# intelligent-environments-lab/CityLearn

Hardware: AMD Instinct MI355X
Metric: building-timesteps/sec at 17 bldgs x 65536 envs; HBM GB/s vs roofline (higher is better)
Workload: dtype f32 (battery soc chain in f64); 1 GPU; citylearn_challenge_2022_phase_all tables (17 buildings, the full year, 8 760 h) x 65536 envs per GPU, cl_step_f32 mode A (one env step per launch, state in HBM, fresh uniform random actions from an 8-tensor ring), env batch sharded over GPUs, no collective; CLD_F64_CHAIN: battery soc chain in float64, degraded capacity carried as the capacity loss; envs_per_gpu=65536, buildings=17, env_pitch=65536, precision=CLD_F64_CHAIN (StepEngine default): 1e-4 free-running over whole episodes, launch=hipGraph replay, reward=RewardFunction, reps=1, statistic=median of reps (each: MAX over ranks)

## Files before the change

citylearn_amd/csrc/cl_kernels.hip:

```cpp
#include "cl_trace.h"
#include "cl_unit.h"
#include "cl_plan.h"
#ifndef CL_LEAN_NT_LOADS
#define CL_LEAN_NT_LOADS true
#endif
#include "cl_philox.h"

#include <type_traits>
#include <mutex>
#include <stdarg.h>
#include <string.h>
#include <stdio.h>

namespace {

int hip_fail(hipError_t e, const char* what) {
    return fail(CL_EHIP, "%s: %s", what, hipGetErrorString(e));
}

hipError_t ensure_dynamic_lds(const void* fn, size_t bytes) {
    struct Seen { const void* fn; int dev; size_t bytes; };
    static Seen seen[64];
    static int n_seen = 0;
    static std::mutex mu;
// ... 154 lines not shown
    for (int j = w; j < opw; j += 16) {
        const int o = by * opw + j;
        if (o >= NQ * TILE || bx * TILE + o % TILE >= a.n_env) continue;
        float pk = 0.0f;
        if (k < a.n_chunks) {
#pragma unroll
            for (int c = 0; c < 4; ++c) pk += k + 16 * c < a.n_chunks ? lds_fold[((k + 16 * c) << sh) + j] : 0.0f;
        }
        float tot = 0.0f;
#pragma unroll
        for (int q = 0; q < 16; ++q) tot += __builtin_bit_cast(float, __builtin_amdgcn_readlane(__builtin_bit_cast(int, pk), q));
        if (lane == 0) a.out_env[(long long)(o / TILE) * a.n_env + bx * TILE + o % TILE] = tot;
    }
}

template <int VEC, bool FLEX = false, bool FOLD = false, bool KPIS = false, bool PRESTORED = false>
CL_DEV void district_reduce(const StepArgs& a, float* lds, int w, int lane, int env0, bool live, long long plane, int rkind,
                            const float (&q_net)[VEC], const float (&q_cost)[VEC], const float (&q_em)[VEC],
                            const float (&q_rw)[VEC], int stride, [[maybe_unused]] const float* lds_fold = nullptr) {
    constexpr int TILE = 64 * VEC;
    const int bx = blockIdx.x, by = blockIdx.y;
    if constexpr (!PRESTORED) {
        float* mine = lds + (size_t)w * NQ * TILE + lane * VEC;
        vstore<VEC>(mine + 0 * TILE, q_net);
        vstore<VEC>(mine + 1 * TILE, q_cost);
        vstore<VEC>(mine + 2 * TILE, q_em);
        vstore<VEC>(mine + 3 * TILE, q_rw);
    }
    const int tile_env0 = bx * TILE;
    [[maybe_unused]] KpiSeries pre;
    if constexpr (KPIS) {
        if (threadIdx.x < TILE && tile_env0 + (int)threadIdx.x < a.n_env) kpi_series_fetch(pre, a.kpi_env + tile_env0 + threadIdx.x, a.n_env);
    }
    __syncthreads();
    const bool coupled = rkind == CLR_MARL || (FLEX && rkind == CLR_EV);
    if (a.n_chunks > 1) {
        float* scratch = a.out_bldg + (long long)CLO_RESERVED * plane;
        const bool deferred = FOLD && a.fused_finish == 2;
        if (deferred) scratch += (long long)(a.t & 1) * a.n_chunks * NQ * a.n_env;
        for (int i = threadIdx.x; i < NQ * TILE; i += blockDim.x) {
            const int q = i / TILE, e = i - q * TILE;
            float s = 0.0f;
            for (int k = 0; k < a.nw; ++k) s += lds[(size_t)k * NQ * TILE + i];
            if (tile_env0 + e < a.n_env) {
                float* dst = scratch + ((long long)by * NQ + q) * a.n_env + tile_env0 + e;
                if (FOLD && a.fused_finish == 1) __hip_atomic_store(dst, s, __ATOMIC_RELAXED, __HIP_MEMORY_SCOPE_AGENT);
                else *dst = s;
            }
        }
        if constexpr (!FOLD) return;
        else {
        if (!a.fused_finish) return;
        if (a.fused_finish == 1 && blockIdx.x == 0 && blockIdx.y == 0 && threadIdx.x == 0)
            reinterpret_cast<unsigned*>(a.out_bldg + (long long)(CLO_RESERVED + 1) * plane - 4)[a.t & 1] = 0u;
        if (a.fused_finish == 2) {
// ... 50 lines not shown
        for (int o = threadIdx.x; o < n_out; o += blockDim.x) {
            const int q = o / TILE, e = o - q * TILE;
            if (tile_env0 + e >= a.n_env) continue;
            float s = 0.0f, sn = 0.0f;
            for (int p = 0; p < rep; ++p) {
                s += part[(size_t)p * n_out + o];
                if (marl) sn += part[(size_t)(rep + p) * n_out + o];
            }
            if (marl && q == CLQ_REWARD) s *= fmaxf(0.0f, sn);
            a.out_env[(long long)q * a.n_env + tile_env0 + e] = s;
        }
        if (threadIdx.x == 0) __hip_atomic_store(ticket, 0u, __ATOMIC_RELAXED, __HIP_MEMORY_SCOPE_AGENT);
        return;
        }
    }
    for (int i = threadIdx.x; i < NQ * TILE; i += blockDim.x) {
        const int q = i / TILE, e = i - q * TILE;
        float s = 0.0f;
        for (int k = 0; k < a.nw; ++k) s += lds[(size_t)k * NQ * TILE + i];
        if (coupled && q == CLQ_REWARD) {
            if (FLEX && rkind == CLR_EV) lds[i] = s;
            continue;
        }
        if (tile_env0 + e < a.n_env) {
            a.out_env[(long long)q * a.n_env + tile_env0 + e] = s;
            if constexpr (KPIS) {
                if (q == CLQ_NET) {
                    if (i == (int)threadIdx.x) kpi_series_apply(a.kpi_env + tile_env0 + e, a.n_env, a.t, s, pre);
                    else kpi_series_update(a.kpi_env + tile_env0 + e, a.n_env, a.t, s);
                }
            }
// ... 35 lines not shown
                    for (int i = 0; i < VEC; ++i) rw[i] = fbi >= 0 ? cl::ev_reward(true, rw[i], n[i], k0[i], kn[i], kp[i]) : 0.0f;
                    if (fbi >= 0 && a.ev_penalty_coef > 0.0f) {
                        float viol[VEC];
                        vload<VEC>(viol, a.flex_out + CLX_VIOLATION * ((long long)a.n_flex_bldg * a.n_env) + (long long)fbi * a.n_env + env0);
#pragma unroll
                        for (int i = 0; i < VEC; ++i) rw[i] -= viol[i] > 0.0f ? viol[i] * a.ev_penalty_coef : 0.0f;
                    }
                }
#pragma unroll
                for (int i = 0; i < VEC; ++i) r_sum[i] += rw[i];
                pstore<VEC, false>(a.out_bldg + CLO_REWARD * plane + off, rw);
            }
        }
        vstore<VEC>(lds + (size_t)w * TILE + lane * VEC, r_sum);
        __syncthreads();
        for (int e = threadIdx.x; e < TILE; e += blockDim.x) {
            float s = 0.0f;
            for (int k = 0; k < a.nw; ++k) s += lds[(size_t)k * TILE + e];
            if (tile_env0 + e < a.n_env) a.out_env[(long long)CLQ_REWARD * a.n_env + tile_env0 + e] = s;
        }
    }
}

template <int VEC, bool FULL, bool DETAIL, bool FLEX = false, int PREC = 0, bool FOLD = false, bool CHECK = false>
__global__ void __launch_bounds__(1024) cl_step_kernel(const StepArgs a) {
    constexpr bool F64 = PREC == 1;
    const int bx = blockIdx.x, by = blockIdx.y;
    extern __shared__ __attribute__((aligned(16))) float lds[];
    constexpr int TILE = 64 * VEC;
    const int lane = threadIdx.x & 63;
    const int w = __builtin_amdgcn_readfirstlane(threadIdx.x >> 6);
// ... 287 lines not shown
            pload<VEC, NTL>(s_eff[m], a.state + CLS_B_EFF * plane + off);
            pload<VEC, NTL>(s_deg[m], a.state + CLS_B_DEGCAP * plane + off);
            if constexpr (F64) {
                pload<VEC, NTL>(s_efl[m], a.state + CLS_B_EFF_LO * plane + off);
                pload<VEC, NTL>(s_dgl[m], a.state + CLS_B_DEGCAP_LO * plane + off);
            }
            if (act_by_bldg) pload<VEC, NTL>(a_es[m], a.actions + (long long)bb[m] * a.act_stride_col + env0);
        }
#pragma unroll
        for (int m = 0; m < 2; ++m) {
            if (m && !own[1]) continue;
            const int b = bb[m];
            cl::Bp B;
            cl::Row R;
            [[maybe_unused]] cl::BattC bc_uni;
            const cl::cl_ctab pb = cl::as_ctab(a.params + (long long)b * CL_NP);
            const cl::cl_ctab qb = cl::as_ctab(a.ts + ((long long)ts_row * a.n_bldg + b) * CL_NF);
            if constexpr (UNI) {
                B.p = a.params + (long long)b * CL_NP; B.flags = CLF_BATTERY; B.a_es = b; B.rw_exponent = 1.0f;
                B.r = cl::pw(pb, CLP_L_TSR);
                cl::load_battc_from(bc_uni, pb);
            } else cl::load_bp_from<false>(B, a.params + (long long)b * CL_NP, pb);
            R.nsl = cl::pw(qb, CLT_NSL); R.sol = cl::pw(qb, CLT_SOLAR); R.price = cl::pw(qb, CLT_PRICE); R.carbon = cl::pw(qb, CLT_CARBON);
            R.outage = false;
            [[maybe_unused]] int od_n = 0, od_col[CL_OBS_FUSED_PER_BLDG], od_src[CL_OBS_FUSED_PER_BLDG];
            [[maybe_unused]] float od_scale[CL_OBS_FUSED_PER_BLDG], od_base[CL_OBS_FUSED_PER_BLDG];
            if constexpr (OBS) {
                const float* __restrict__ trow = of->table + (size_t)(of->row + (ts_row - a.t)) * of->n_cols;
                const int d0 = of->start[b];
                od_n = of->start[b + 1] - d0;
#pragma unroll
                for (int k = 0; k < CL_OBS_FUSED_PER_BLDG; ++k) {
                    const int d = min(d0 + min(k, max(od_n - 1, 0)), CLOB_MAX_DEPS - 1);
                    od_col[k] = of->deps[d].col; od_src[k] = of->deps[d].src; od_scale[k] = of->deps[d].scale;
                    od_base[k] = trow[od_col[k]];
                }
// ... 25 lines not shown
                    cl::unit_step<false>(B, R, a.t, quirk, act, S, O);
                    if (FLEX && fbi >= 0) cl::apply_flex(false, R.price, R.carbon, x_load[i], 0.0f, O);
                    const float rw = cl::unit_reward<false>(rkind, B, S, O.net);
                    s_soc[m][i] = S.soc; s_eff[m][i] = S.eff; s_deg[m][i] = S.degcap;
                    o_net[i] = O.net; o_rw[i] = rw;
                    q_net[i] += O.net; q_cost[i] += O.cost; q_em[i] += O.emission;
                    q_rw[i] += (FLEX && rkind == CLR_EV) ? cl::marl_reward(O.net, 1.0f) : rw;
                }
            } else {
                const bool first = quirk && a.t == 0;
                float c_ns = first ? 3.0f * R.nsl : R.nsl;
                float sol = R.sol;
                const float cbk = first ? 2.0f : 1.0f;
                CL_PIN_V(c_ns); CL_PIN_V(sol);
                if constexpr (UNI) {
                    __builtin_amdgcn_sched_barrier(0);
#pragma unroll
                    for (int i = 0; i < VEC; ++i) CL_PIN_V(a_es[m][i]);
                }
                float soc_rw[VEC];
                if (F64 && batt) {
                    if constexpr (F64) {
                        cl::BattP64 B64;
                        cl::load_batt64(B64, B.p);
                        if (B.a_es < 0) {
#pragma unroll
                            for (int i = 0; i < VEC; ++i) a_es[m][i] = 0.0f;
                        }
#pragma unroll
                        for (int i = 0; i < VEC; ++i) {
// ... 5 lines not shown
                            o_net[i] = fmaf(c_ns + o_cb[i], B.r, sol);
                        }
                    }
                } else if (PREC == 2 && batt) {
                    if constexpr (PREC == 2) {
                        cl::BattC bc;
                        if constexpr (UNI) bc = bc_uni;
                        else cl::load_battc_from(bc, pb);
                        if (no_es) {
#pragma unroll
                            for (int i = 0; i < VEC; ++i) a_es[m][i] = 0.0f;
                        }
#pragma unroll
                        for (int i = 0; i < VEC; ++i) {
                            cl::State S = {s_soc[m][i], s_eff[m][i], s_deg[m][i], 0.0f, 0.0f, 0.0f};
                            const float eb = cl::battery_charge_chain(bc, a_es[m][i], INFINITY, S);
                            s_soc[m][i] = S.soc; s_eff[m][i] = S.eff; s_deg[m][i] = S.degcap;
                            soc_rw[i] = S.soc;
                            o_cb[i] = cbk * eb;
                            o_net[i] = fmaf(c_ns + o_cb[i], B.r, sol);
                        }
                    }
                } else if (batt) {
                    cl::BattP Bv = B.batt;
                    CL_PIN_V(Bv.cpc_a0); CL_PIN_V(Bv.cpc_b0); CL_PIN_V(Bv.cpc_a1); CL_PIN_V(Bv.cpc_b1);
                    CL_PIN_V(Bv.pec_a0); CL_PIN_V(Bv.pec_b0); CL_PIN_V(Bv.pec_a1); CL_PIN_V(Bv.pec_b1);
                    CL_PIN_V(Bv.pec_a2); CL_PIN_V(Bv.pec_b2); CL_PIN_V(Bv.pec_a3); CL_PIN_V(Bv.pec_b3);
                    if (no_es) {
#pragma unroll
                        for (int i = 0; i < VEC; ++i) a_es[m][i] = 0.0f;
                    }
// ... 86 lines not shown
    if constexpr (OBS) {
        if (w == 0) {
            float* tile = lds + (size_t)a.nw * NQ * TILE;
            for (int c = of->n_cols; c < of->pitch; ++c) {
#pragma unroll
                for (int i = 0; i < VEC; ++i) tile[(size_t)(lane * VEC + i) * of->pitch + c] = 0.0f;
            }
        }
    }
    CL_TRACE_AFTER(13, q_net[0]);
    [[maybe_unused]] KpiSeries base_pre;
    [[maybe_unused]] const bool base_writer = KPI && !FLEX && threadIdx.x == blockDim.x - 1 && (blockIdx.x * TILE) % CL_ROW0_BLOCK == 0;
    if constexpr (KPI && !FLEX) {
        if (base_writer) kpi_series_fetch(base_pre, a.kpi_env + (long long)CLKE_PER_COND * a.n_env + blockIdx.x * TILE, a.n_env);
    }
    district_reduce<VEC, FLEX, false, KPI && !FLEX>(a, lds, w, lane, env0, live, plane, rkind, q_net, q_cost, q_em, q_rw, a.nw);
    if constexpr (KPI && !FLEX) {
        if (base_writer) {
            float sum = 0.0f;
            for (int b = 0; b < a.n_bldg; ++b) sum += lds[(size_t)a.nw * NQ * TILE + b];
            kpi_series_apply(a.kpi_env + (long long)CLKE_PER_COND * a.n_env + blockIdx.x * TILE, a.n_env, a.t, sum, base_pre);
        }
    }
    if constexpr (OBS) {
        typedef float f4 __attribute__((ext_vector_type(4)));
        const int tile_env0 = blockIdx.x * TILE;
        const int rows = min(TILE, a.n_env - tile_env0);
        const f4* src4 = reinterpret_cast<const f4*>(lds + (size_t)a.nw * NQ * TILE);
        f4* dst4 = reinterpret_cast<f4*>(of->obs + (size_t)tile_env0 * of->pitch);
        const int total4 = rows * of->pitch / 4;
        for (int q = threadIdx.x; q < total4; q += blockDim.x) {
// ... 109 lines not shown
#pragma unroll
        for (int i = 0; i < VEC; ++i) {
            float act_v = 0.0f;
            if (B.a_es >= 0) act_v = act_by_bldg ? a_es[b][i] : a.actions[(long long)B.a_es * a.act_stride_col + (long long)(env + i) * a.act_stride_env];
            cl::State S;
            S.soc = batt ? s_soc[b][i] : 0.0f; S.eff = batt ? s_eff[b][i] : 1.0f; S.degcap = batt ? s_deg[b][i] : 0.0f;
            S.cs = S.hs = S.ds = 0.0f;
            const cl::Act act = {0.0f, 0.0f, 0.0f, act_v, 0.0f, 0.0f};
            cl::Out O;
            if constexpr (PREC == 2) {
                float eb = 0.0f;
                if (batt) {
                    cl::BattC bc;
                    cl::load_battc64(bc, &sp[b][0] + (PW + 4) - CLP_C_FIRST);
                    bc.cap32 = B.batt.cap; bc.omd32 = B.batt.omd; bc.degk = B.batt.degk;
                    eb = cl::battery_charge_chain(bc, act_v, INFINITY, S);
                }
                const bool first = quirk && a.t == 0;
                const float c_ns = first ? 3.0f * R.nsl : R.nsl, c_b = first ? 2.0f * eb : eb;
                O.net = fmaf(c_ns + c_b, B.r, R.sol); O.cost = cl::mul_rn(O.net, R.price); O.emission = fmaxf(0.0f, O.net * R.carbon);
            } else cl::unit_step<false>(B, R, a.t, quirk, act, S, O);
            o_soc[i] = S.soc; o_eff[i] = S.eff; o_deg[i] = S.degcap; o_net[i] = O.net;
            o_rw[i] = cl::unit_reward<false>(rkind, B, S, O.net);
            s_soc[b][i] = O.net;
            q_net[i] += O.net; q_cost[i] += O.cost; q_em[i] += O.emission; q_rw[i] += o_rw[i];
        }
        if (batt) {
            pstore<VEC, NT>(a.state + CLS_B_SOC * plane + off, o_soc);
            pstore<VEC, NT>(a.state + CLS_B_EFF * plane + off, o_eff);
            pstore<VEC, NT>(a.state + CLS_B_DEGCAP * plane + off, o_deg);
        }
// ... 1048 lines not shown
```

citylearn_amd/csrc/cl_policy.h:

```cpp
#pragma once
#include "cl_policy_common.h"

#ifdef __HIPCC__
namespace {

constexpr int CLPOL_MAX_H = 32;
constexpr int CLPOL_ROW = 3 * CLPOL_MAX_H + 8;

constexpr size_t rollout_policy_lds_floats(int nw, int tile) { return (size_t)nw * NQ * tile + (size_t)nw * 2 * CLPOL_ROW; }

template <int VEC, int PREC>
__global__ void __launch_bounds__(1024) cl_rollout_policy_kernel(const PolicyArgs p) {
    extern __shared__ __attribute__((aligned(16))) float lds[];
    constexpr int MB = 2, TILE = 64 * VEC;
    const RolloutArgs& r = p.r;
    const StepArgs& a = r.s;
    const int lane = threadIdx.x & 63;
    const int w = __builtin_amdgcn_readfirstlane(threadIdx.x >> 6);
    const int tile_env0 = blockIdx.x * TILE;
    const int env0 = tile_env0 + lane * VEC;
    const bool live = env0 < a.n_env;
    const long long plane = (long long)a.n_bldg * a.n_env;
    const int rkind = (a.flags & CLD_REWARD_MASK) >> CLD_REWARD_SHIFT;
    const bool quirk = a.flags & CLD_REF_T0_QUIRK;
// ... 126 lines not shown

            const bool first = quirk && t == 0;
            float c_ns = first ? 3.0f * R.nsl : R.nsl, sol = R.sol;
            const float cbk = first ? 2.0f : 1.0f;
            if constexpr (VEC > 1) { CL_PIN_V(c_ns); CL_PIN_V(sol); }
            const bool batt = B[m].flags & CLF_BATTERY;
            float nets[VEC], socs[VEC], rws[VEC];
            [[maybe_unused]] cl::BattC bc;
            if constexpr (PREC == 2) {
                if (batt) load_battc_const(bc, as_const(B[m].p));
            }
#pragma unroll
            for (int i = 0; i < VEC; ++i) {
                float eb = 0.0f;
                if constexpr (PREC == 2) {
                    if (batt) eb = cl::battery_charge_chain(bc, a_es[i], INFINITY, St[m][i]);
                } else if (batt) eb = cl::battery_energy(Bv[m], a_es[i] * Bv[m].pdt, St[m][i]);
                nets[i] = fmaf(c_ns + cbk * eb, B[m].r, sol);
                socs[i] = St[m][i].soc;
            }
            cl::lean_rewards<VEC>(rkind, B[m], socs, nets, rws);
#pragma unroll
            for (int i = 0; i < VEC; ++i) {
                last_net[m][i] = nets[i]; last_rw[m][i] = rws[i];
                q_net[i] += nets[i]; q_cost[i] += cl::mul_rn(nets[i], R.price); q_em[i] += fmaxf(0.0f, nets[i] * R.carbon); q_rw[i] += rws[i];
            }
            if (tr && live) {
                float* const tb = tr + off[m];
                vstore<VEC>(tb + (long long)CLPOL_T_ACTION * plane, a_es);
                vstore<VEC>(tb + (long long)CLPOL_T_NET * plane, nets);
                vstore<VEC>(tb + (long long)CLPOL_T_SOC * plane, socs);
// ... 81 lines not shown
```

citylearn_amd/csrc/cl_policy_central.h:

```cpp
#pragma once
#include "cl_policy_common.h"

#ifdef __HIPCC__
namespace {

constexpr int CLPCA_ROW = CLPCA_MAX_HIDDEN + 8;

constexpr size_t rollout_policy_central_lds_floats(int nw, int n_bldg, int h) {
    return (size_t)nw * NQ * 64 + (size_t)2 * n_bldg * 64 + (size_t)h * 64 + (size_t)2 * h * n_bldg + (size_t)nw * 2 * CLPCA_ROW;
}

template <int PREC>
__global__ void __launch_bounds__(1024) cl_rollout_policy_central_kernel(const PolicyArgs p) {
    extern __shared__ __attribute__((aligned(16))) float lds[];
    constexpr int MB = 2, VEC = 1, TILE = 64;
    const RolloutArgs& r = p.r;
    const StepArgs& a = r.s;
    const int lane = threadIdx.x & 63;
    const int w = __builtin_amdgcn_readfirstlane(threadIdx.x >> 6);
    const int tile_env0 = blockIdx.x * TILE;
    const int env0 = tile_env0 + lane;
    const bool live = env0 < a.n_env;
    const long long plane = (long long)a.n_bldg * a.n_env;
    const int rkind = (a.flags & CLD_REWARD_MASK) >> CLD_REWARD_SHIFT;
// ... 142 lines not shown
            }

            const bool first = quirk && t == 0;
            float c_ns = first ? 3.0f * R.nsl : R.nsl, sol = R.sol;
            const float cbk = first ? 2.0f : 1.0f;
            const bool batt = B[m].flags & CLF_BATTERY;
            float nets[VEC], socs[VEC], rws[VEC];
            [[maybe_unused]] cl::BattC bc;
            if constexpr (PREC == 2) {
                if (batt) load_battc_const(bc, as_const(B[m].p));
            }
#pragma unroll
            for (int i = 0; i < VEC; ++i) {
                float eb = 0.0f;
                if constexpr (PREC == 2) {
                    if (batt) eb = cl::battery_charge_chain(bc, a_es[i], INFINITY, St[m][i]);
                } else if (batt) eb = cl::battery_energy(Bv[m], a_es[i] * Bv[m].pdt, St[m][i]);
                nets[i] = fmaf(c_ns + cbk * eb, B[m].r, sol);
                socs[i] = St[m][i].soc;
            }
            cl::lean_rewards<VEC>(rkind, B[m], socs, nets, rws);
#pragma unroll
            for (int i = 0; i < VEC; ++i) {
                last_net[m][i] = nets[i]; last_rw[m][i] = rws[i];
                q_net[i] += nets[i]; q_cost[i] += cl::mul_rn(nets[i], R.price); q_em[i] += fmaxf(0.0f, nets[i] * R.carbon); q_rw[i] += rws[i];
            }
            X[(size_t)bidx[m] * TILE + lane] = socs[0];
            X[(size_t)(NB + bidx[m]) * TILE + lane] = nets[0];
            if (tr && live) {
                float* const tb = tr + off[m];
                vstore<VEC>(tb + (long long)CLPOL_T_ACTION * plane, a_es);
// ... 74 lines not shown
```

citylearn_amd/csrc/cl_policy_chunk.h:

```cpp
#pragma once
#include "cl_policy.h"

#ifdef __HIPCC__
namespace {

constexpr size_t rollout_policy_chunk_lds_floats(int nw, int tile) { return (size_t)nw * NQ * tile + (size_t)nw * 2 * CLPOL_ROW; }

template <int VEC, int PREC>
__global__ void __launch_bounds__(1024) cl_rollout_policy_chunk_kernel(const PolicyArgs p) {
    extern __shared__ __attribute__((aligned(16))) float lds[];
    constexpr int MB = 2, TILE = 64 * VEC;
    const RolloutArgs& r = p.r;
    const StepArgs& a = r.s;
    const int lane = threadIdx.x & 63;
    const int w = __builtin_amdgcn_readfirstlane(threadIdx.x >> 6);
    const int tile_env0 = blockIdx.x * TILE;
    const int env0 = tile_env0 + lane * VEC;
    const bool live = env0 < a.n_env;
    const long long plane = (long long)a.n_bldg * a.n_env;
    const int rkind = (a.flags & CLD_REWARD_MASK) >> CLD_REWARD_SHIFT;
    const bool quirk = a.flags & CLD_REF_T0_QUIRK;
    const int H = p.n_hidden;
    const int blk = tile_env0 / CL_ROW0_BLOCK;
    const int row0 = a.env_row0 ? a.env_row0[blk] : 0;
// ... 126 lines not shown

            const bool first = quirk && t == 0;
            float c_ns = first ? 3.0f * R.nsl : R.nsl, sol = R.sol;
            const float cbk = first ? 2.0f : 1.0f;
            if constexpr (VEC > 1) { CL_PIN_V(c_ns); CL_PIN_V(sol); }
            const bool batt = B[m].flags & CLF_BATTERY;
            float nets[VEC], socs[VEC], rws[VEC];
            [[maybe_unused]] cl::BattC bc;
            if constexpr (PREC == 2) {
                if (batt) load_battc_const(bc, as_const(B[m].p));
            }
#pragma unroll
            for (int i = 0; i < VEC; ++i) {
                float eb = 0.0f;
                if constexpr (PREC == 2) {
                    if (batt) eb = cl::battery_charge_chain(bc, a_es[i], INFINITY, St[m][i]);
                } else if (batt) eb = cl::battery_energy(Bv[m], a_es[i] * Bv[m].pdt, St[m][i]);
                nets[i] = fmaf(c_ns + cbk * eb, B[m].r, sol);
                socs[i] = St[m][i].soc;
            }
            cl::lean_rewards<VEC>(rkind, B[m], socs, nets, rws);
#pragma unroll
            for (int i = 0; i < VEC; ++i) {
                last_net[m][i] = nets[i]; last_rw[m][i] = rws[i];
                q_net[i] += nets[i]; q_cost[i] += cl::mul_rn(nets[i], R.price); q_em[i] += fmaxf(0.0f, nets[i] * R.carbon); q_rw[i] += rws[i];
            }
            if (tr && live) {
                float* const tb = tr + off[m];
                vstore<VEC>(tb + (long long)CLPOL_T_ACTION * plane, a_es);
                vstore<VEC>(tb + (long long)CLPOL_T_NET * plane, nets);
                vstore<VEC>(tb + (long long)CLPOL_T_SOC * plane, socs);
// ... 47 lines not shown
```

citylearn_amd/csrc/cl_policy_deep.h:

```cpp
#pragma once
#include "cl_policy_common.h"

#ifdef __HIPCC__
namespace {

constexpr int CLPD_MAX_H = 32;
constexpr int CLPD_TAIL = 8;

constexpr int clpd_row_floats(int h1, int h2) { return 2 * h1 + (h1 + 1) * h2 + h2 + CLPD_TAIL; }

struct DeepPolicyArgs {
    PolicyArgs p;
    const float* __restrict__ l2;
    int n_hidden2;
};

constexpr int CLPD_M_WN = 32, CLPD_M_B2 = 64, CLPD_M_W3 = 96, CLPD_M_TAIL = 128, CLPD_M_FRAG = 136;
constexpr int CLPD_M_FRAG_FLOATS = 2 * 2 * 64 * 4;
constexpr int CLPD_M_ROW = CLPD_M_FRAG + CLPD_M_FRAG_FLOATS;
constexpr int CLPD_M_L2 = CLPD_M_FRAG_FLOATS + CLPD_MAX_H + 4;

typedef _Float16 clpd_f16x8 __attribute__((ext_vector_type(8)));
typedef float clpd_f32x16 __attribute__((ext_vector_type(16)));

// ... 272 lines not shown

            const bool first = quirk && t == 0;
            float c_ns = first ? 3.0f * R.nsl : R.nsl, sol = R.sol;
            const float cbk = first ? 2.0f : 1.0f;
            if constexpr (VEC > 1) { CL_PIN_V(c_ns); CL_PIN_V(sol); }
            const bool batt = B[m].flags & CLF_BATTERY;
            float nets[VEC], socs[VEC], rws[VEC];
            [[maybe_unused]] cl::BattC bc;
            if constexpr (PREC == 2) {
                if (batt) load_battc_const(bc, as_const(B[m].p));
            }
#pragma unroll
            for (int i = 0; i < VEC; ++i) {
                float eb = 0.0f;
                if constexpr (PREC == 2) {
                    if (batt) eb = cl::battery_charge_chain(bc, a_es[i], INFINITY, St[m][i]);
                } else if (batt) eb = cl::battery_energy(Bv[m], a_es[i] * Bv[m].pdt, St[m][i]);
                nets[i] = fmaf(c_ns + cbk * eb, B[m].r, sol);
                socs[i] = St[m][i].soc;
            }
            cl::lean_rewards<VEC>(rkind, B[m], socs, nets, rws);
#pragma unroll
            for (int i = 0; i < VEC; ++i) {
                last_net[m][i] = nets[i]; last_rw[m][i] = rws[i];
                q_net[i] += nets[i]; q_cost[i] += cl::mul_rn(nets[i], R.price); q_em[i] += fmaxf(0.0f, nets[i] * R.carbon); q_rw[i] += rws[i];
            }
            if (tr && live) {
                float* const tb = tr + off[m];
                vstore<VEC>(tb + (long long)CLPOL_T_ACTION * plane, a_es);
                vstore<VEC>(tb + (long long)CLPOL_T_NET * plane, nets);
                vstore<VEC>(tb + (long long)CLPOL_T_SOC * plane, socs);
// ... 64 lines not shown
```

citylearn_amd/csrc/cl_policy_kpi.h:

```cpp
#pragma once

#ifdef __HIPCC__
namespace {

constexpr size_t rollout_policy_kpi_lds_floats(int nw, int tile) { return rollout_kpi_lds_floats(nw, tile) + (size_t)nw * 2 * CLPOL_ROW; }

constexpr bool clpk_pins(int vec, int prec) { return vec == 1; }

template <int VEC, int PREC>
__global__ void __launch_bounds__(1024) cl_rollout_policy_kpi_kernel(const PolicyArgs p) {
    extern __shared__ __attribute__((aligned(16))) float lds[];
    constexpr int MB = 2, TILE = 64 * VEC, S = CL_RKPI_S;
    const RolloutArgs& r = p.r;
    const StepArgs& a = r.s;
    const int lane = threadIdx.x & 63;
    const int w = __builtin_amdgcn_readfirstlane(threadIdx.x >> 6);
    const int tile_env0 = blockIdx.x * TILE;
    const int env0 = tile_env0 + lane * VEC;
    const bool live = env0 < a.n_env;
    const long long plane = (long long)a.n_bldg * a.n_env;
    const int rkind = (a.flags & CLD_REWARD_MASK) >> CLD_REWARD_SHIFT;
    const bool quirk = a.flags & CLD_REF_T0_QUIRK;
    const int H = p.n_hidden;
    const int blk = tile_env0 / CL_ROW0_BLOCK;
// ... 158 lines not shown
            if (head && lane == 0) {
                float* brw = brow + (size_t)slot * 4 * CL_RKPI_NB + w + m * a.nw;
                brw[0 * CL_RKPI_NB] = fmaf(c_ns, B[m].r, sol); brw[1 * CL_RKPI_NB] = R.carbon; brw[2 * CL_RKPI_NB] = R.price; brw[3 * CL_RKPI_NB] = R.nsl;
            }
            if constexpr (VEC > 1) { CL_PIN_V(c_ns); CL_PIN_V(sol); }
            const bool batt = B[m].flags & CLF_BATTERY;
            float nets[VEC], socs[VEC], rws[VEC];
            [[maybe_unused]] cl::BattC bc;
            if constexpr (PREC == 2) {
                if (batt) load_battc_const(bc, as_const(B[m].p));
            }
#pragma unroll
            for (int i = 0; i < VEC; ++i) {
                float eb = 0.0f;
                if constexpr (PREC == 2) {
                    if (batt) eb = cl::battery_charge_chain(bc, a_es[i], INFINITY, St[m][i]);
                } else if (batt) eb = cl::battery_energy(Bv[m], a_es[i] * Bv[m].pdt, St[m][i]);
                nets[i] = fmaf(c_ns + cbk * eb, B[m].r, sol);
                socs[i] = St[m][i].soc;
            }
            cl::lean_rewards<VEC>(rkind, B[m], socs, nets, rws);
#pragma unroll
            for (int i = 0; i < VEC; ++i) {
                last_net[m][i] = nets[i]; last_rw[m][i] = rws[i];
                q_net[i] += nets[i]; q_cost[i] += cl::mul_rn(nets[i], R.price); q_em[i] += fmaxf(0.0f, nets[i] * R.carbon); q_rw[i] += rws[i];
                k_pos[m][i] += fmaxf(nets[i], 0.0f); k_net[m][i] += nets[i];
                k_em[m][i] += fmaxf(nets[i] * R.carbon, 0.0f); k_cost[m][i] += fmaxf(nets[i] * R.price, 0.0f);
            }
            if (tr && live) {
                float* const tb = tr + off[m];
                vstore<VEC>(tb + (long long)CLPOL_T_ACTION * plane, a_es);
// ... 126 lines not shown
```

citylearn_amd/csrc/cl_rollout.h:

```cpp
#pragma once

#include "cl_philox.h"

#ifdef __HIPCC__
namespace {

struct RolloutArgs {
    StepArgs s;
    long long act_stride_step;
    const float* __restrict__ act_low;
    const float* __restrict__ act_high;
    float* __restrict__ ret_env;
    unsigned long long seed;
    int t0, k_steps;
};

struct PhiloxCache { uint32_t w0, w1, w2, w3; };
template <int VEC>
CL_DEV void rollout_action_cached(float (&dst)[VEC], PhiloxCache (&cache)[VEC], const RolloutArgs& r, int col, int env0, int t, int k, bool live);

template <int VEC>
CL_DEV void rollout_action(float (&dst)[VEC], const RolloutArgs& r, int col, int env0, int t, int k, bool live) {
    if (col < 0 || (r.s.actions && !live)) {
#pragma unroll
// ... 129 lines not shown
            if constexpr (!FULL) {
                const bool first = quirk && t == 0;
                float c_ns = first ? 3.0f * R.nsl : R.nsl, sol = R.sol;
                const float cbk = first ? 2.0f : 1.0f;
                if constexpr (VEC > 1) { CL_PIN_V(c_ns); CL_PIN_V(sol); }
                const bool batt = B[m].flags & CLF_BATTERY;
                float nets[VEC], socs[VEC], rws[VEC];
                [[maybe_unused]] cl::BattC bc;
                if constexpr (PREC == 2) {
                    if (batt) cl::load_battc(bc, B[m].p);
                }
#pragma unroll
                for (int i = 0; i < VEC; ++i) {
                    float eb = 0.0f;
                    if constexpr (PREC == 2) {
                        if (batt) eb = cl::battery_charge_chain(bc, a_es[i], INFINITY, S[m][i]);
                    } else if (batt) eb = cl::battery_energy(Bv[m], a_es[i] * Bv[m].pdt, S[m][i]);
                    nets[i] = fmaf(c_ns + cbk * eb, B[m].r, sol);
                    socs[i] = S[m][i].soc;
                }
                cl::lean_rewards<VEC>(rkind, B[m], socs, nets, rws);
#pragma unroll
                for (int i = 0; i < VEC; ++i) {
                    last[m][i].net = nets[i]; last_rw[m][i] = rws[i];
                    q_net[i] += nets[i]; q_cost[i] += cl::mul_rn(nets[i], R.price); q_em[i] += fmaxf(0.0f, nets[i] * R.carbon); q_rw[i] += rws[i];
                }
            } else {
#pragma unroll
                for (int i = 0; i < VEC; ++i) {
                    const cl::Act act = {a_cs[i], a_hs[i], a_ds[i], a_es[i], a_cd[i], a_hd[i]};
                    cl::unit_step<FULL, PREC>(B[m], R, t, quirk, act, S[m][i], last[m][i]);
// ... 272 lines not shown
            if (head && lane == 0) {
                float* row = brow + (size_t)slot * 4 * CL_RKPI_NB + w + m * a.nw;
                row[0 * CL_RKPI_NB] = fmaf(c_ns, B[m].r, sol); row[1 * CL_RKPI_NB] = R.carbon; row[2 * CL_RKPI_NB] = R.price; row[3 * CL_RKPI_NB] = R.nsl;
            }
            if constexpr (VEC > 1) { CL_PIN_V(c_ns); CL_PIN_V(sol); }
            const bool batt = B[m].flags & CLF_BATTERY;
            float nets[VEC], socs[VEC], rws[VEC];
            [[maybe_unused]] cl::BattC bc;
            if constexpr (PREC == 2) {
                if (batt) load_battc_const(bc, as_const(B[m].p));
            }
#pragma unroll
            for (int i = 0; i < VEC; ++i) {
                float eb = 0.0f;
                if constexpr (PREC == 2) {
                    if (batt) eb = cl::battery_charge_chain(bc, a_es[i], INFINITY, St[m][i]);
                } else if (batt) eb = cl::battery_energy(Bv[m], a_es[i] * Bv[m].pdt, St[m][i]);
                nets[i] = fmaf(c_ns + cbk * eb, B[m].r, sol);
                socs[i] = St[m][i].soc;
            }
            cl::lean_rewards<VEC>(rkind, B[m], socs, nets, rws);
#pragma unroll
            for (int i = 0; i < VEC; ++i) {
                last_net[m][i] = nets[i]; last_rw[m][i] = rws[i];
                q_net[i] += nets[i]; q_cost[i] += cl::mul_rn(nets[i], R.price); q_em[i] += fmaxf(0.0f, nets[i] * R.carbon); q_rw[i] += rws[i];
                k_pos[m][i] += fmaxf(nets[i], 0.0f); k_net[m][i] += nets[i];
                k_em[m][i] += fmaxf(nets[i] * R.carbon, 0.0f); k_cost[m][i] += fmaxf(nets[i] * R.price, 0.0f);
            }
        }
        vstore<VEC>(lds + ((size_t)slot * a.nw + w) * TILE + lane * VEC, q_net);
        if (rkind == CLR_MARL) {
// ... 358 lines not shown
```

citylearn_amd/csrc/cl_unit.h:

```cpp
#pragma once

#include <stdint.h>
#include "../../include/citylearn_amd.h"

#ifdef CL_HOST_SHIM
#include <math.h>
#include <string.h>
#define CL_DEV inline
namespace cl {
inline float rcp(float x) { return 1.0f / x; }
inline float rsq(float x) { return 1.0f / sqrtf(x); }
inline float fsqrt(float x) { return sqrtf(x); }
inline float med3(float a, float b, float c) { return fmaxf(fminf(a, b), fminf(fmaxf(a, b), c)); }
inline float __uint_as_float(uint32_t u) { float f; memcpy(&f, &u, 4); return f; }
inline float __powf(float a, float b) { return powf(a, b); }
}
#else
#include <hip/hip_runtime.h>
#define CL_DEV __device__ __forceinline__
namespace cl {
CL_DEV float rcp(float x) { return __builtin_amdgcn_rcpf(x); }
CL_DEV float rsq(float x) { return __builtin_amdgcn_rsqf(x); }
CL_DEV float fsqrt(float x) { return __builtin_amdgcn_sqrtf(x); }
CL_DEV float med3(float a, float b, float c) { return __builtin_amdgcn_fmed3f(a, b, c); }
// ... 286 lines not shown
CL_DEV void load_battc64(BattC& C, const uint32_t* __restrict__ p) { load_battc64_from(C, p); }

template <class P>
CL_DEV void load_battc_from(BattC& C, P p) {
    load_battc64_from(C, p);
    C.cap32 = pw(p, CLP_L_CAP); C.omd32 = pw(p, CLP_L_OMD); C.degk = pw(p, CLP_L_DEGK);
}
CL_DEV void load_battc(BattC& C, const uint32_t* __restrict__ p) { load_battc_from(C, p); }

CL_DEV double rsq64(double x) {
    const double y = (double)rsq((float)x);
    const double e = __builtin_fma(-(0.5 * x) * y, y, 0.5);
    return __builtin_fma(y, e, y);
}

CL_DEV float battery_charge_chain(const BattC& C, float a_es, float flex, State& S) {
    const float prev = S.soc;
    const double e_init = fmax(0.0, (double)(prev * C.cap32) * C.oml);
    const double socn = e_init * C.rcap;
    const double pmax = __builtin_fma(C.cdb1, fmax(socn - C.cx1, 0.0), __builtin_fma(C.cb0, socn, C.ca0));
    const double E = fmin((double)a_es * C.pdt, (double)flex);
    const double degcap = C.cap - (double)S.degcap;
    const double e_chg = fmin(fmin(pmax, C.pow), fmin(degcap - e_init, E));
    const double lim = fmax((double)((prev - C.omd32) * C.cap32 * fsqrt(S.eff)), 0.0);
    const double e_dis = fmax(fmax(-pmax, -lim), E);
    const bool chg = E >= 0.0;
    double e = chg ? e_chg : e_dis;
    const double x = fmin(fabs(E), pmax) * C.rpow;
    double eff = __builtin_fma(C.eb0, x, C.ea0);
    eff = __builtin_fma(C.edb1, fmax(x - C.ex1, 0.0), eff);
    eff = __builtin_fma(C.edb2, fmax(x - C.ex2, 0.0), eff);
    eff = __builtin_fma(C.edb3, fmax(x - C.ex3, 0.0), eff);
    const double irte = rsq64(eff), rte = eff * irte;
    e *= C.r;
    const bool chg_e = e >= 0.0;
    const double e_fin = fmin(fmax(__builtin_fma(e, chg_e ? rte : irte, e_init), 0.0), C.cap);
    const double d = e_fin - e_init;
    const float eb = (float)(d * (chg_e ? irte : rte));
    const float degcap32 = C.cap32 - S.degcap;
    S.degcap = fminf(fmaf(C.degk * fabsf(eb), rcp(fmaxf(degcap32, CL_ZDP)), S.degcap), C.cap32);
    S.eff = (float)eff;
    S.soc = (float)(e_fin * C.rcap);
    return eb;
}

CL_DEV void tank_charge(float e, float prev_soc, float cap, float capl, float rte, float irte, float icap,
                        float maxin, float maxout, float r, float& soc, float& eb) {
    e *= r;
    e = e >= 0.0f ? fminf(e, maxin) : fmaxf(-maxout, e);
    e *= r;
    const float e_init = fmaxf(0.0f, prev_soc * capl);
    const float e_fin = e >= 0.0f ? fminf(fmaf(e, rte, e_init), cap) : fmaxf(0.0f, fmaf(e, irte, e_init));
    soc = e_fin * icap;
    const float d = e_fin - e_init;
    eb = d * (d >= 0.0f ? irte : rte);
}

template <bool CHECK = false>
CL_DEV void end_use(const Bp& B, const Row& R, Acc& A, float& c, float demand, float a_sto, float cscale,
                    float dev_pow, float cop, float icop, const TankP& T, float ir, float& soc, float& eb, float& e_dev,
// ... 28 lines not shown
    const double energy = fmin((double)a_es * bp.pow * bp.dt, (double)flex);
    return battery_charge_ref(bp, energy / bp.r, first, S);
}

template <bool FULL, int PREC = 0, bool CHECK = false>
CL_DEV void unit_step(const Bp& B, const Row& R, int t, bool t0_quirk, const Act& a, State& S, Out& O) {
    constexpr bool F64 = PREC == 1;
    [[maybe_unused]] uint32_t viol = 0u;
    const bool first = t0_quirk && t == 0;
    const bool has_batt = B.flags & CLF_BATTERY;
    if constexpr (!FULL) {
        float eb = 0.0f;
        if constexpr (F64) {
            if (has_batt) eb = battery_step_f64(B.p, a.es, INFINITY, t == 0, S);
        } else if constexpr (PREC == 2) {
            if (has_batt) { BattC bc; load_battc(bc, B.p); eb = battery_charge_chain(bc, a.es, INFINITY, S); }
        } else if (has_batt) eb = battery_step(B.batt, a.es, INFINITY, S);
        const float c_ns = first ? 3.0f * R.nsl : R.nsl;
        const float c_b = first ? 2.0f * eb : eb;
        if constexpr (CHECK) { if (!(R.nsl >= 0.0f)) viol |= CLV_NSL; O.viol = viol; }
        const float net = fmaf(c_ns + c_b, B.r, R.sol);
        O.net = net; O.cost = mul_rn(net, R.price); O.emission = fmaxf(0.0f, net * R.carbon);
        O.eb = eb; O.cool_dem = 0.0f; O.heat_dem = 0.0f; O.dhw_dem = 0.0f; O.c_cool = 0.0f; O.c_heat = 0.0f; O.c_dhw = 0.0f; O.c_ns = c_ns * B.r;
        O.base_net = net - c_b * B.r; O.net_ws = O.base_net; O.expected = R.nsl; O.served = R.nsl;
        O.se_cool = O.se_heat = O.se_dhw = 0.0f;
        return;
    } else {
        Acc A = {0.0f, 0.0f, 0.0f, 0.0f, 0.0f};
        const bool heat_hp = B.flags & CLF_HEAT_IS_HP;
        const float t0_iheat = heat_hp ? R.icop_h : B.t0_iheat_div;
        if (first) {
// ... 156 lines not shown
```

Before: 156.1 billion building-timesteps/s.

## Add straight reduce tail, prefetch second building params, drop infinite flex clamp

Adds a specialised district-reduce tail for the plain lean launch that sums the per-wave LDS rows with a fixed 16-load unrolled pattern, keeps the stride and destination pointer in scalar or precomputed registers, and writes through a global address-space pointer. In the uniform battery path it also issues early scalar loads of the second building's parameter and timeseries cache lines to warm them. A flex-less overload of battery_charge_chain skips the min against infinity. Together these aim to trim instruction and latency overhead in the tail and the battery chain, at the cost of extra code paths and scalar registers.

```diff
diff --git a/citylearn_amd/csrc/cl_kernels.hip b/citylearn_amd/csrc/cl_kernels.hip
--- a/citylearn_amd/csrc/cl_kernels.hip
+++ b/citylearn_amd/csrc/cl_kernels.hip
@@ -192,10 +192,23 @@
     }
 }
 
-template <int VEC, bool FLEX = false, bool FOLD = false, bool KPIS = false, bool PRESTORED = false>
+template <bool ALL, int ROW>
+CL_DEV float wave_rows_sum(const float* col, int nw) {
+    float v[16];
+#pragma unroll
+    for (int k = 0; k < 16; ++k) v[k] = col[(size_t)(ALL ? k : min(k, nw - 1)) * ROW];
+    asm volatile("" : "+v"(v[0]), "+v"(v[1]), "+v"(v[2]), "+v"(v[3]), "+v"(v[4]), "+v"(v[5]), "+v"(v[6]), "+v"(v[7]),
+                      "+v"(v[8]), "+v"(v[9]), "+v"(v[10]), "+v"(v[11]), "+v"(v[12]), "+v"(v[13]), "+v"(v[14]), "+v"(v[15]));
+    float s = 0.0f;
+#pragma unroll
+    for (int k = 0; k < 16; ++k) s += (ALL || k < nw) ? v[k] : 0.0f;
+    return s;
+}
+template <int VEC, bool FLEX = false, bool FOLD = false, bool KPIS = false, bool PRESTORED = false, bool STRAIGHT = false>
 CL_DEV void district_reduce(const StepArgs& a, float* lds, int w, int lane, int env0, bool live, long long plane, int rkind,
                             const float (&q_net)[VEC], const float (&q_cost)[VEC], const float (&q_em)[VEC],
                             const float (&q_rw)[VEC], int stride, [[maybe_unused]] const float* lds_fold = nullptr) {
+    static_assert(!STRAIGHT || (!KPIS && !FOLD && !PRESTORED), "the straight tail is the plain lean launches'");
     constexpr int TILE = 64 * VEC;
     const int bx = blockIdx.x, by = blockIdx.y;
     if constexpr (!PRESTORED) {
@@ -210,13 +223,44 @@
     if constexpr (KPIS) {
         if (threadIdx.x < TILE && tile_env0 + (int)threadIdx.x < a.n_env) kpi_series_fetch(pre, a.kpi_env + tile_env0 + threadIdx.x, a.n_env);
     }
+    const bool coupled = rkind == CLR_MARL || (FLEX && rkind == CLR_EV);
+    [[maybe_unused]] bool straight = false;
+    [[maybe_unused]] int st_step = 0, st_nenv = 0;
+    [[maybe_unused]] unsigned long long st_dst = 0ull;
+    if constexpr (STRAIGHT) {
+        straight = !(a.n_chunks > 1) && !coupled;
+        st_step = 64 * a.nw; st_nenv = a.n_env;
+        st_dst = (unsigned long long)(a.out_env + (long long)((int)threadIdx.x / TILE) * a.n_env + tile_env0 + (int)threadIdx.x % TILE);
+        asm volatile("" : "+s"(st_step), "+s"(st_nenv), "+v"(st_dst));
+    }
     __syncthreads();
-    const bool coupled = rkind == CLR_MARL || (FLEX && rkind == CLR_EV);
+    auto bdim = [&]() -> int { if constexpr (STRAIGHT) return st_step; else return (int)blockDim.x; };
+    if constexpr (STRAIGHT) {
+        if (__builtin_expect(straight, 1)) {
+            typedef float __attribute__((address_space(1))) gfloat;
+            const int nw = st_step >> 6;
+            auto tail = [&](auto all) {
+                for (int i = threadIdx.x; i < NQ * TILE; i += st_step) {
+                    const int q = i / TILE, e = i - q * TILE;
+                    const float s = wave_rows_sum<decltype(all)::value, NQ * TILE>(lds + i, nw);
+                    if (tile_env0 + e < st_nenv) {
+                        const int q0 = (int)threadIdx.x / TILE, e0 = (int)threadIdx.x - q0 * TILE;
+                        gfloat* dst = (gfloat*)st_dst;
+                        if (i != (int)threadIdx.x) dst += (long long)(q - q0) * st_nenv + (e - e0);
+                        *dst = s;
+                    }
+                }
+            };
+            if (__builtin_expect(nw == 16, 1)) tail(std::true_type{});
+            else tail(std::false_type{});
+            return;
+        }
+    }
     if (a.n_chunks > 1) {
         float* scratch = a.out_bldg + (long long)CLO_RESERVED * plane;
         const bool deferred = FOLD && a.fused_finish == 2;
         if (deferred) scratch += (long long)(a.t & 1) * a.n_chunks * NQ * a.n_env;
-        for (int i = threadIdx.x; i < NQ * TILE; i += blockDim.x) {
+        for (int i = threadIdx.x; i < NQ * TILE; i += bdim()) {
             const int q = i / TILE, e = i - q * TILE;
             float s = 0.0f;
             for (int k = 0; k < a.nw; ++k) s += lds[(size_t)k * NQ * TILE + i];
@@ -297,7 +341,7 @@
         return;
         }
     }
-    for (int i = threadIdx.x; i < NQ * TILE; i += blockDim.x) {
+    for (int i = threadIdx.x; i < NQ * TILE; i += bdim()) {
         const int q = i / TILE, e = i - q * TILE;
         float s = 0.0f;
         for (int k = 0; k < a.nw; ++k) s += lds[(size_t)k * NQ * TILE + i];
@@ -363,7 +407,7 @@
         }
         vstore<VEC>(lds + (size_t)w * TILE + lane * VEC, r_sum);
         __syncthreads();
-        for (int e = threadIdx.x; e < TILE; e += blockDim.x) {
+        for (int e = threadIdx.x; e < TILE; e += bdim()) {
             float s = 0.0f;
             for (int k = 0; k < a.nw; ++k) s += lds[(size_t)k * TILE + e];
             if (tile_env0 + e < a.n_env) a.out_env[(long long)CLQ_REWARD * a.n_env + tile_env0 + e] = s;
@@ -681,12 +725,24 @@
             cl::Bp B;
             cl::Row R;
             [[maybe_unused]] cl::BattC bc_uni;
+            [[maybe_unused]] uint32_t warm[6] = {0u, 0u, 0u, 0u, 0u, 0u};
             const cl::cl_ctab pb = cl::as_ctab(a.params + (long long)b * CL_NP);
             const cl::cl_ctab qb = cl::as_ctab(a.ts + ((long long)ts_row * a.n_bldg + b) * CL_NF);
             if constexpr (UNI) {
                 B.p = a.params + (long long)b * CL_NP; B.flags = CLF_BATTERY; B.a_es = b; B.rw_exponent = 1.0f;
                 B.r = cl::pw(pb, CLP_L_TSR);
                 cl::load_battc_from(bc_uni, pb);
+                if (m == 0) {
+                    const int b1 = bb[own[1] ? 1 : 0];
+                    const cl::cl_ctab pb1 = cl::as_ctab(a.params + (long long)b1 * CL_NP);
+                    const cl::cl_ctab qb1 = cl::as_ctab(a.ts + ((long long)ts_row * a.n_bldg + b1) * CL_NF);
+                    constexpr int c_lines = (2 * CLPC_PEC_DB3 + 1) / 16 + 1;
+                    static_assert(c_lines == 3 && CLP_C_FIRST % 16 == 0 && CLP_L_TSR / 16 == CLP_L_DEGK / 16, "the lines the second building's group reads");
+#pragma unroll
+                    for (int k = 0; k < c_lines; ++k) warm[k] = pb1[CLP_C_FIRST + 16 * k];
+                    warm[3] = pb1[CLP_L_TSR];
+                    warm[4] = qb1[CLT_NSL]; warm[5] = qb1[CLT_PRICE];
+                }
             } else cl::load_bp_from<false>(B, a.params + (long long)b * CL_NP, pb);
             R.nsl = cl::pw(qb, CLT_NSL); R.sol = cl::pw(qb, CLT_SOLAR); R.price = cl::pw(qb, CLT_PRICE); R.carbon = cl::pw(qb, CLT_CARBON);
             R.outage = false;
@@ -742,6 +798,7 @@
                 const float cbk = first ? 2.0f : 1.0f;
                 CL_PIN_V(c_ns); CL_PIN_V(sol);
                 if constexpr (UNI) {
+                    if (m == 0) asm volatile("" :: "s"(warm[0]), "s"(warm[1]), "s"(warm[2]), "s"(warm[3]), "s"(warm[4]), "s"(warm[5]));
                     __builtin_amdgcn_sched_barrier(0);
 #pragma unroll
                     for (int i = 0; i < VEC; ++i) CL_PIN_V(a_es[m][i]);
@@ -777,7 +834,7 @@
 #pragma unroll
                         for (int i = 0; i < VEC; ++i) {
                             cl::State S = {s_soc[m][i], s_eff[m][i], s_deg[m][i], 0.0f, 0.0f, 0.0f};
-                            const float eb = cl::battery_charge_chain(bc, a_es[m][i], INFINITY, S);
+                            const float eb = cl::battery_charge_chain(bc, a_es[m][i], S);
                             s_soc[m][i] = S.soc; s_eff[m][i] = S.eff; s_deg[m][i] = S.degcap;
                             soc_rw[i] = S.soc;
                             o_cb[i] = cbk * eb;
@@ -894,7 +951,7 @@
     if constexpr (KPI && !FLEX) {
         if (base_writer) kpi_series_fetch(base_pre, a.kpi_env + (long long)CLKE_PER_COND * a.n_env + blockIdx.x * TILE, a.n_env);
     }
-    district_reduce<VEC, FLEX, false, KPI && !FLEX>(a, lds, w, lane, env0, live, plane, rkind, q_net, q_cost, q_em, q_rw, a.nw);
+    district_reduce<VEC, FLEX, false, KPI && !FLEX, false, !KPI>(a, lds, w, lane, env0, live, plane, rkind, q_net, q_cost, q_em, q_rw, a.nw);
     if constexpr (KPI && !FLEX) {
         if (base_writer) {
             float sum = 0.0f;
@@ -1034,7 +1091,7 @@
                     cl::BattC bc;
                     cl::load_battc64(bc, &sp[b][0] + (PW + 4) - CLP_C_FIRST);
                     bc.cap32 = B.batt.cap; bc.omd32 = B.batt.omd; bc.degk = B.batt.degk;
-                    eb = cl::battery_charge_chain(bc, act_v, INFINITY, S);
+                    eb = cl::battery_charge_chain(bc, act_v, S);
                 }
                 const bool first = quirk && a.t == 0;
                 const float c_ns = first ? 3.0f * R.nsl : R.nsl, c_b = first ? 2.0f * eb : eb;
diff --git a/citylearn_amd/csrc/cl_policy.h b/citylearn_amd/csrc/cl_policy.h
--- a/citylearn_amd/csrc/cl_policy.h
+++ b/citylearn_amd/csrc/cl_policy.h
@@ -164,7 +164,7 @@
             for (int i = 0; i < VEC; ++i) {
                 float eb = 0.0f;
                 if constexpr (PREC == 2) {
-                    if (batt) eb = cl::battery_charge_chain(bc, a_es[i], INFINITY, St[m][i]);
+                    if (batt) eb = cl::battery_charge_chain(bc, a_es[i], St[m][i]);
                 } else if (batt) eb = cl::battery_energy(Bv[m], a_es[i] * Bv[m].pdt, St[m][i]);
                 nets[i] = fmaf(c_ns + cbk * eb, B[m].r, sol);
                 socs[i] = St[m][i].soc;
diff --git a/citylearn_amd/csrc/cl_policy_central.h b/citylearn_amd/csrc/cl_policy_central.h
--- a/citylearn_amd/csrc/cl_policy_central.h
+++ b/citylearn_amd/csrc/cl_policy_central.h
@@ -180,7 +180,7 @@
             for (int i = 0; i < VEC; ++i) {
                 float eb = 0.0f;
                 if constexpr (PREC == 2) {
-                    if (batt) eb = cl::battery_charge_chain(bc, a_es[i], INFINITY, St[m][i]);
+                    if (batt) eb = cl::battery_charge_chain(bc, a_es[i], St[m][i]);
                 } else if (batt) eb = cl::battery_energy(Bv[m], a_es[i] * Bv[m].pdt, St[m][i]);
                 nets[i] = fmaf(c_ns + cbk * eb, B[m].r, sol);
                 socs[i] = St[m][i].soc;
diff --git a/citylearn_amd/csrc/cl_policy_chunk.h b/citylearn_amd/csrc/cl_policy_chunk.h
--- a/citylearn_amd/csrc/cl_policy_chunk.h
+++ b/citylearn_amd/csrc/cl_policy_chunk.h
@@ -164,7 +164,7 @@
             for (int i = 0; i < VEC; ++i) {
                 float eb = 0.0f;
                 if constexpr (PREC == 2) {
-                    if (batt) eb = cl::battery_charge_chain(bc, a_es[i], INFINITY, St[m][i]);
+                    if (batt) eb = cl::battery_charge_chain(bc, a_es[i], St[m][i]);
                 } else if (batt) eb = cl::battery_energy(Bv[m], a_es[i] * Bv[m].pdt, St[m][i]);
                 nets[i] = fmaf(c_ns + cbk * eb, B[m].r, sol);
                 socs[i] = St[m][i].soc;
diff --git a/citylearn_amd/csrc/cl_policy_deep.h b/citylearn_amd/csrc/cl_policy_deep.h
--- a/citylearn_amd/csrc/cl_policy_deep.h
+++ b/citylearn_amd/csrc/cl_policy_deep.h
@@ -310,7 +310,7 @@
             for (int i = 0; i < VEC; ++i) {
                 float eb = 0.0f;
                 if constexpr (PREC == 2) {
-                    if (batt) eb = cl::battery_charge_chain(bc, a_es[i], INFINITY, St[m][i]);
+                    if (batt) eb = cl::battery_charge_chain(bc, a_es[i], St[m][i]);
                 } else if (batt) eb = cl::battery_energy(Bv[m], a_es[i] * Bv[m].pdt, St[m][i]);
                 nets[i] = fmaf(c_ns + cbk * eb, B[m].r, sol);
                 socs[i] = St[m][i].soc;
diff --git a/citylearn_amd/csrc/cl_policy_kpi.h b/citylearn_amd/csrc/cl_policy_kpi.h
--- a/citylearn_amd/csrc/cl_policy_kpi.h
+++ b/citylearn_amd/csrc/cl_policy_kpi.h
@@ -196,7 +196,7 @@
             for (int i = 0; i < VEC; ++i) {
                 float eb = 0.0f;
                 if constexpr (PREC == 2) {
-                    if (batt) eb = cl::battery_charge_chain(bc, a_es[i], INFINITY, St[m][i]);
+                    if (batt) eb = cl::battery_charge_chain(bc, a_es[i], St[m][i]);
                 } else if (batt) eb = cl::battery_energy(Bv[m], a_es[i] * Bv[m].pdt, St[m][i]);
                 nets[i] = fmaf(c_ns + cbk * eb, B[m].r, sol);
                 socs[i] = St[m][i].soc;
diff --git a/citylearn_amd/csrc/cl_rollout.h b/citylearn_amd/csrc/cl_rollout.h
--- a/citylearn_amd/csrc/cl_rollout.h
+++ b/citylearn_amd/csrc/cl_rollout.h
@@ -167,7 +167,7 @@
                 for (int i = 0; i < VEC; ++i) {
                     float eb = 0.0f;
                     if constexpr (PREC == 2) {
-                        if (batt) eb = cl::battery_charge_chain(bc, a_es[i], INFINITY, S[m][i]);
+                        if (batt) eb = cl::battery_charge_chain(bc, a_es[i], S[m][i]);
                     } else if (batt) eb = cl::battery_energy(Bv[m], a_es[i] * Bv[m].pdt, S[m][i]);
                     nets[i] = fmaf(c_ns + cbk * eb, B[m].r, sol);
                     socs[i] = S[m][i].soc;
@@ -470,7 +470,7 @@
             for (int i = 0; i < VEC; ++i) {
                 float eb = 0.0f;
                 if constexpr (PREC == 2) {
-                    if (batt) eb = cl::battery_charge_chain(bc, a_es[i], INFINITY, St[m][i]);
+                    if (batt) eb = cl::battery_charge_chain(bc, a_es[i], St[m][i]);
                 } else if (batt) eb = cl::battery_energy(Bv[m], a_es[i] * Bv[m].pdt, St[m][i]);
                 nets[i] = fmaf(c_ns + cbk * eb, B[m].r, sol);
                 socs[i] = St[m][i].soc;
diff --git a/citylearn_amd/csrc/cl_unit.h b/citylearn_amd/csrc/cl_unit.h
--- a/citylearn_amd/csrc/cl_unit.h
+++ b/citylearn_amd/csrc/cl_unit.h
@@ -324,12 +324,14 @@
     return __builtin_fma(y, e, y);
 }
 
-CL_DEV float battery_charge_chain(const BattC& C, float a_es, float flex, State& S) {
+template <bool CLAMP = true>
+CL_DEV float battery_charge_chain(const BattC& C, float a_es, [[maybe_unused]] float flex, State& S) {
     const float prev = S.soc;
     const double e_init = fmax(0.0, (double)(prev * C.cap32) * C.oml);
     const double socn = e_init * C.rcap;
     const double pmax = __builtin_fma(C.cdb1, fmax(socn - C.cx1, 0.0), __builtin_fma(C.cb0, socn, C.ca0));
-    const double E = fmin((double)a_es * C.pdt, (double)flex);
+    double E = (double)a_es * C.pdt;
+    if constexpr (CLAMP) E = fmin(E, (double)flex);
     const double degcap = C.cap - (double)S.degcap;
     const double e_chg = fmin(fmin(pmax, C.pow), fmin(degcap - e_init, E));
     const double lim = fmax((double)((prev - C.omd32) * C.cap32 * fsqrt(S.eff)), 0.0);
@@ -354,6 +356,8 @@
     return eb;
 }
 
+CL_DEV float battery_charge_chain(const BattC& C, float a_es, State& S) { return battery_charge_chain<false>(C, a_es, 0.0f, S); }
+
 CL_DEV void tank_charge(float e, float prev_soc, float cap, float capl, float rte, float irte, float icap,
                         float maxin, float maxout, float r, float& soc, float& eb) {
     e *= r;
@@ -412,7 +416,7 @@
         if constexpr (F64) {
             if (has_batt) eb = battery_step_f64(B.p, a.es, INFINITY, t == 0, S);
         } else if constexpr (PREC == 2) {
-            if (has_batt) { BattC bc; load_battc(bc, B.p); eb = battery_charge_chain(bc, a.es, INFINITY, S); }
+            if (has_batt) { BattC bc; load_battc(bc, B.p); eb = battery_charge_chain(bc, a.es, S); }
         } else if (has_batt) eb = battery_step(B.batt, a.es, INFINITY, S);
         const float c_ns = first ? 3.0f * R.nsl : R.nsl;
         const float c_b = first ? 2.0f * eb : eb;
```

Result: faster. 157.9 billion building-timesteps/s (median of 6 runs) (+1.1%).
